# ShawnHymel/ei-keyword-spotting

Measured on AMD Instinct MI355X. Metric: 1s@16kHz clips/sec (MFCC+CNN), higher is better.
Workload: dtype f32

## Files before the change

### ei-keyword-spotting_amd/csrc/kws_fast.hip

```cpp
#include <atomic>

#include "kws_device.h"
#include "kws_fast.h"
#include "kws_bfly_m2k1.h"
#include "kws_fast_maxmin.h"
#if KWS_FAST_WPS >= 3
#define kws_fast_kernel kws_fast_kernel_w3
#define kws_launch_fast kws_launch_fast_w3
#define kws_launch_fast_prof kws_launch_fast_prof_w3
#endif
#include "kws_nn_int8_dev.h"

typedef float v4f __attribute__((ext_vector_type(4)));
#if KWS_FAST_WPS >= 3
#define KWS_OPAQUE3(v) asm volatile("" : "+v"(v))
#define KWS_LANE3(lane) ((int)__builtin_amdgcn_mbcnt_hi(~0u, __builtin_amdgcn_mbcnt_lo(~0u, 0u)))
#define KWS_FAST_SINK (shared + FP.sink_off)
#else
#define KWS_OPAQUE3(v) do { } while (0)
#define KWS_LANE3(lane) (lane)
#define KWS_FAST_SINK (F + FP.sink_off)
#endif
static_assert(KWS_FAST_ZF == KWS_ZF && KWS_FAST_WAVE == KWS_WAVE, "kws_fast.h mirrors kws_device.h");

// ... 514 lines not shown
    const unsigned inv = k.inv_ocp20;
    const int sstride = k.stage_stride, out_w = k.out_w, out_c = k.out_c, pool = k.pool, pstr = k.pool_stride;
    const float pmin = k.pool_min, pmax = k.pool_max;
    if (!pooled) {
        const int npad = out_cp - out_c;
        if (npad == 0) return;
        const unsigned pinv = k.inv_npad20;
        for (int i = lane; i < k.pool_w * npad; i += KWS_WAVE) {
            const int p = (int)(((unsigned)i * pinv) >> 20), c = out_c + (i - p * npad);
            img[p * out_stride + c] = 0.0f;
        }
        return;
    }
    for (int i0 = 0; i0 < items; i0 += 2 * KWS_WAVE) {
        float v[2][8];
        int p[2], c[2];
#pragma unroll
        for (int u = 0; u < 2; ++u) {
            const int i = min(i0 + u * KWS_WAVE + lane, items - 1);
            p[u] = (int)(((unsigned)i * inv) >> 20);
            c[u] = i - p[u] * out_cp;
            const float *sp = stage + p[u] * pstr * sstride + min(c[u], out_c - 1);
#pragma unroll
            for (int j = 0; j < 8; ++j) {
                const int r = (j < pool) ? min(p[u] * pstr + j, out_w - 1) : p[u] * pstr;
                v[u][j] = sp[(r - p[u] * pstr) * sstride];
            }
        }
#pragma unroll
        for (int u = 0; u < 2; ++u) {
            float m = v[u][0];
#pragma unroll
            for (int j = 1; j < 8; ++j) m = fast_max(m, v[u][j]);
            m = fast_clamp_u(m, pmin, pmax);
            if (i0 + u * KWS_WAVE + lane < items) img[p[u] * out_stride + c[u]] = c[u] < out_c ? m : 0.0f;
        }
    }
}

template <int TAPS>
__device__ __forceinline__ void fast_dw_t(const KwsFastBlock &k, const float *__restrict__ in, float *__restrict__ img,
                                          const float *__restrict__ shared, int lane, int out_stride, int out_cp)
{
    const int out_c = k.out_c, in_w = k.in_w, out_w = k.out_w, pad_left = k.pad_left, in_stride = k.in_stride, mult = k.mult;
    const bool pooled = k.pool > 1 || k.pool_stride > 1;
    const int n_seg = pooled ? k.pool_w : k.dw_nseg;
    const int seg_rows = pooled ? k.pool : k.dw_seg_rows, seg_step = pooled ? k.pool_stride : seg_rows;
    const int items = n_seg * out_cp;
    const unsigned inv = k.inv_ocp20;
    const float cmin = k.conv_min, cmax = k.conv_max, amin = k.add_min, amax = k.add_max, pmin = k.pool_min, pmax = k.pool_max;
    const bool has_add = k.has_add != 0;
    const float *wt = shared + k.w_off;
    for (int i = lane; i < items; i += KWS_WAVE) {
        const int seg = (int)(((unsigned)i * inv) >> 20), c = i - seg * out_cp, cc = min(c, out_c - 1);
        const float *col = in + (mult == 1 ? cc : cc / mult);
        float w[TAPS];
#pragma unroll
        for (int t = 0; t < TAPS; ++t) w[t] = wt[t * out_c + cc];
        const float bias = shared[k.bias_off + cc], addc = shared[k.addc_off + cc];
        const int r0 = seg * seg_step, r1 = min(r0 + seg_rows, out_w);
        auto fetch = [&](int row) { const float v = col[min(max(row, 0), in_w - 1) * in_stride]; return (unsigned)row < (unsigned)in_w ? v : 0.0f; };
        float x[TAPS + 3];
#pragma unroll
        for (int t = 0; t + 1 < TAPS; ++t) x[t] = fetch(r0 + t - pad_left);
        float m = -FLT_MAX;
        float *dst = img + c;
        for (int r = r0; r < r1; r += 4) {
#pragma unroll
            for (int e = 0; e < 4; ++e) x[TAPS - 1 + e] = fetch(r + e + TAPS - 1 - pad_left);
#pragma unroll
            for (int e = 0; e < 4; ++e) {
                float acc = 0.0f;
#pragma unroll
                for (int t = 0; t < TAPS; ++t) acc = __fmaf_rn(x[e + t], w[t], acc);
                float v = fminf(fmaxf(acc + bias, cmin), cmax);
                if (has_add) v = fminf(fmaxf(v + addc, amin), amax);
                const bool live = r + e < r1;
                if (pooled) m = live ? fmaxf(m, v) : m;
                else if (live) dst[(r + e) * out_stride] = c < out_c ? v : 0.0f;
            }
#pragma unroll
            for (int t = 0; t + 1 < TAPS; ++t) x[t] = x[t + 4];
        }
        if (pooled) dst[seg * out_stride] = c < out_c ? fminf(fmaxf(m, pmin), pmax) : 0.0f;
    }
}

__device__ __forceinline__ void fast_dwconv_any(const KwsFastBlock &k, const float *__restrict__ in, float *__restrict__ img,
                                                const float *__restrict__ shared, int lane, int out_stride, int out_cp)
{
    const int items = k.pool_w * out_cp, out_c = k.out_c, in_w = k.in_w, out_w = k.out_w, taps = k.taps, pad_left = k.pad_left;
    const int in_stride = k.in_stride, pool = k.pool, pstr = k.pool_stride, mult = k.mult;
    const unsigned inv = k.inv_ocp20;
    const float cmin = k.conv_min, cmax = k.conv_max, amin = k.add_min, amax = k.add_max, pmin = k.pool_min, pmax = k.pool_max;
    const bool has_add = k.has_add != 0;
    const float *wt = shared + k.w_off;
    for (int i = lane; i < items; i += KWS_WAVE) {
        const int p = (int)(((unsigned)i * inv) >> 20), c = i - p * out_cp, cc = min(c, out_c - 1);
        const float *col = in + (mult == 1 ? cc : cc / mult);
        const float bias = shared[k.bias_off + cc], addc = shared[k.addc_off + cc];
        float m = -FLT_MAX;
        for (int j = 0; j < pool; ++j) {
            const int r = p * pstr + j;
            if (r >= out_w) break;
            float acc = 0.0f;
            for (int tap = 0; tap < taps; ++tap) {
                const int row = r + tap - pad_left;
                if ((unsigned)row < (unsigned)in_w) acc = __fmaf_rn(col[row * in_stride], wt[tap * out_c + cc], acc);
            }
            float v = fminf(fmaxf(acc + bias, cmin), cmax);
            if (has_add) v = fminf(fmaxf(v + addc, amin), amax);
            m = fmaxf(m, v);
        }
        m = fminf(fmaxf(m, pmin), pmax);
        img[p * out_stride + c] = c < out_c ? m : 0.0f;
    }
}

__device__ __forceinline__ void fast_dwconv(const KwsFastBlock &k, const float *__restrict__ in, float *__restrict__ img,
                                            const float *__restrict__ shared, int lane, int out_stride, int out_cp)
{
    switch (k.taps) {
    case 1: fast_dw_t<1>(k, in, img, shared, lane, out_stride, out_cp); break;
    case 2: fast_dw_t<2>(k, in, img, shared, lane, out_stride, out_cp); break;
    case 3: fast_dw_t<3>(k, in, img, shared, lane, out_stride, out_cp); break;
    case 4: fast_dw_t<4>(k, in, img, shared, lane, out_stride, out_cp); break;
    case 5: fast_dw_t<5>(k, in, img, shared, lane, out_stride, out_cp); break;
    case 6: fast_dw_t<6>(k, in, img, shared, lane, out_stride, out_cp); break;
    case 7: fast_dw_t<7>(k, in, img, shared, lane, out_stride, out_cp); break;
    case 8: fast_dw_t<8>(k, in, img, shared, lane, out_stride, out_cp); break;
    default: fast_dwconv_any(k, in, img, shared, lane, out_stride, out_cp); break;
    }
}

template <int CR, int CG, bool DEFER, bool SPLIT = false, int SAFE = 0>
__device__ __forceinline__ float fast_cmvn(float *__restrict__ img, const float *__restrict__ cnt_tab, const int *__restrict__ upd, int fs,
                                           float inv_win, const float *__restrict__ guard_tab, float level, float abs_scale, bool silent, float sys_t2, int piv_row, const float *__restrict__ mref, bool c0_exact, int lane, int nfr, int ncep,
                                           const float *__restrict__ ext_tab, float *__restrict__ sink, int in_cp = 0)
{
    static_assert(!SPLIT || (DEFER && CG == 16), "the split store is written for column blocks of 16 and the deferred guard sum");
    static_assert(SAFE == 0 || (SPLIT && SAFE <= CR), "rows known to be live: the split form only");
    constexpr int NG = KWS_WAVE / CG;
    const int cgrp = min(lane / CG, NG - 1), cl = lane - (lane / CG) * CG;
    const bool lane_on = SPLIT || lane < NG * CG;
#define CMVN_ROW_LIVE(r0v, i) ((i) < SAFE || (r0v) + (i) < nfr)
#define CMVN_ROW(r0v, i) ((i) < SAFE ? (r0v) + (i) : min((r0v) + (i), nfr - 1))
    const int r0 = cgrp * CR;
    const int nfr8 = (nfr + 7) & ~7;
    const float *cnt = cnt_tab + cgrp * nfr8;
    float vacc = 0.0f;
    int u[CR - 1];
    int xo[KWS_FAST_CMVN_EXT];
    float we[KWS_FAST_CMVN_EXT], m0 = 0.0f;
#if KWS_FAST_WPS < 3
#pragma unroll
    for (int i = 0; i < CR - 1; ++i) u[i] = upd[min(r0 + i, nfr - 1)];
    if (ext_tab) {
        const float *ext = ext_tab + cgrp * (1 + 2 * KWS_FAST_CMVN_EXT);
        m0 = ext[0];
#pragma unroll
        for (int e = 0; e < KWS_FAST_CMVN_EXT; ++e) { xo[e] = __float_as_int(ext[1 + 2 * e]); we[e] = ext[2 + 2 * e]; }
    }
#endif
    for (int cb = 0; cb < ncep; cb += CG) {
#if KWS_FAST_WPS >= 3
        {
            int cg_ = cgrp;
            KWS_OPAQUE3(cg_);
            const int r0_ = cg_ * CR;
#pragma unroll
            for (int i = 0; i < CR - 1; ++i) u[i] = upd[CMVN_ROW(r0_, i)];
            if (ext_tab) {
                const float *ext = ext_tab + cg_ * (1 + 2 * KWS_FAST_CMVN_EXT);
                m0 = ext[0];
#pragma unroll
                for (int e = 0; e < KWS_FAST_CMVN_EXT; ++e) { xo[e] = __float_as_int(ext[1 + 2 * e]); we[e] = ext[2 + 2 * e]; }
            }
        }
#endif
        const int c = cb + cl;
        const bool act = lane_on && c < ncep && (SAFE > 0 || r0 < nfr);
        float *col = img + min(c, ncep - 1);
        const float piv = col[(ext_tab ? piv_row : min(r0 + CR / 2, nfr - 1)) * fs];
        const float4 gcol = ((const float4 *)guard_tab)[cb + cl];
        const bool is_c0 = c0_exact && cb + cl == 0;
        float g_abs = __fmaf_rn(gcol.y, level, gcol.x * abs_scale);
        if constexpr (SPLIT) g_abs = act ? g_abs : 0.0f;
        float g_rel = (cb + cl == 0 ? c0_exact : silent) ? gcol.w : gcol.z;
        float mr[CR];
#pragma unroll
        for (int i = 0; i < CR; ++i) mr[i] = (c0_exact && cb == 0) ? mref[CMVN_ROW(r0, i)] : 0.0f;
        float own[CR];
#pragma unroll
        for (int i = 0; i < CR; ++i) own[i] = col[CMVN_ROW(r0, i) * fs];
        float dl[CR - 1], da[CR - 1];
#pragma unroll
        for (int i = 0; i < CR - 1; ++i) { dl[i] = col[u[i] & 0xffff]; da[i] = col[(unsigned)u[i] >> 16]; }
        float S0 = 0.0f, S1 = 0.0f, Q0 = 0.0f, Q1 = 0.0f;
        if (ext_tab) {
            float xe[KWS_FAST_CMVN_EXT];
#pragma unroll
            for (int e = 0; e < KWS_FAST_CMVN_EXT; ++e) xe[e] = col[xo[e]];
            float T0 = 0.0f, T1 = 0.0f, U0 = 0.0f, U1 = 0.0f;
#pragma unroll
            for (int i = 0; i < CR; ++i) {
                const float d = (lane_on && CMVN_ROW_LIVE(r0, i)) ? own[i] - piv : 0.0f;
                if (i & 1) { T1 += d; U1 = __fmaf_rn(d, d, U1); } else { T0 += d; U0 = __fmaf_rn(d, d, U0); }
            }
            float T = T0 + T1, U = U0 + U1;
            float Tt = T, Ut = U;
#pragma unroll
            for (int g = 1; g < NG; ++g) {
                const int src = (cl + CG * ((cgrp + g) % NG)) << 2;
                Tt += __int_as_float(__builtin_amdgcn_ds_bpermute(src, __float_as_int(T)));
                Ut += __int_as_float(__builtin_amdgcn_ds_bpermute(src, __float_as_int(U)));
            }
            S0 = m0 * Tt; Q0 = m0 * Ut;
#pragma unroll
            for (int e = 0; e < KWS_FAST_CMVN_EXT; ++e) {
                const float d = xe[e] - piv, wd = we[e] * d;
                S1 += wd;
                Q1 = __fmaf_rn(wd, d, Q1);
            }
        } else
        for (int j0 = 0; j0 < nfr8; j0 += 8) {
            float x[8];
#pragma unroll
            for (int e = 0; e < 8; ++e) x[e] = col[min(j0 + e, nfr - 1) * fs];
            const float4 wa = *(const float4 *)(cnt + j0), wb = *(const float4 *)(cnt + j0 + 4);
            const float w[8] = { wa.x, wa.y, wa.z, wa.w, wb.x, wb.y, wb.z, wb.w };
#pragma unroll
            for (int e = 0; e < 8; e += 2) {
                const float d0 = x[e] - piv, d1 = x[e + 1] - piv;
                const float wd0 = w[e] * d0, wd1 = w[e + 1] * d1;
                S0 += wd0; S1 += wd1;
                Q0 = __fmaf_rn(wd0, d0, Q0); Q1 = __fmaf_rn(wd1, d1, Q1);
            }
        }
#pragma unroll
        for (int i = 0; i < CR - 1; ++i) { dl[i] -= piv; da[i] -= piv; }
        float S = S0 + S1, Q = Q0 + Q1;
        if constexpr (DEFER) {
            const float m0 = S * inv_win, v0 = fmaxf(__fmaf_rn(-m0, m0, Q * inv_win), 0.0f), am0 = m0 + piv;
            g_rel = (cb + cl != 0 && v0 < sys_t2 * (am0 * am0)) ? gcol.w : g_rel;
            if constexpr (SPLIT) g_rel = act ? g_rel : 0.0f;
        }
        float o[CR], gq[DEFER ? CR : 1];
#pragma unroll
        for (int i = 0; i < CR; ++i) {
            const float m = S * inv_win;
            float var = __fmaf_rn(-m, m, Q * inv_win);
            var = fmaxf(var, 0.0f);
            const float sd = __builtin_amdgcn_sqrtf(var);
            const float rstd = __builtin_amdgcn_rcpf(sd + FLT_EPSILON);
            const float gterm = __fmaf_rn(g_rel, fabsf(m + piv), g_abs) * rstd;
            if constexpr (DEFER) gq[i] = gterm;
            else vacc = (act && r0 + i < nfr) ? __fmaf_rn(gterm, gterm, vacc) : vacc;
            o[i] = (is_c0 ? own[i] - mr[i] : (own[i] - piv) - m) * rstd;
            if (i + 1 < CR) {
                S = (S + da[i]) - dl[i];
                Q = __fmaf_rn(da[i], da[i], Q);
                Q = __fmaf_rn(-dl[i], dl[i], Q);
            }
        }
        WAVE_SYNC();
        if constexpr (SPLIT) {
            _Float16 *const hcol = (_Float16 *)((char *)img + 4 * cb) + cl;
            const bool col_on = lane_on && c < in_cp;
            _Float16 *dst_i = col_on ? hcol + r0 * (2 * fs) : (_Float16 *)sink;
            const int dst_step = col_on ? 2 * fs : 0;
            float sc = c < ncep ? (float)(1 << KWS_SPLIT22_PRE_EXP) : 0.0f;
#pragma unroll
            for (int i = 0; i < CR; ++i) asm volatile("" : "+v"(o[i]));
#pragma unroll
            for (int i = 0; i < CR; ++i) {
                const bool live = CMVN_ROW_LIVE(r0, i);
                _Float16 hi, lo;
                const float d = kws_split22(o[i], sc, &hi, &lo);
                _Float16 *const dst = live ? dst_i : (_Float16 *)sink;
                dst[0] = hi;
                dst[KWS_FAST_PRE_LO / 2] = lo;
                dst_i += dst_step;
                sc = __fmaf_rn(d, 0.0f, sc);
                vacc = live ? __fmaf_rn(gq[i], gq[i], vacc) : vacc;
            }
            vacc = (SAFE > 0 || r0 < nfr) ? __fmaf_rn(sc, 0.0f, vacc) : vacc;
        } else {
#pragma unroll
        for (int i = 0; i < CR; ++i) {
            const int r = r0 + i;
            const bool live = act && r < nfr;
            *(live ? col + r * fs : sink) = o[i];
            if constexpr (DEFER) vacc = live ? __fmaf_rn(gq[i], gq[i], vacc) : vacc;
        }
        }
    }
    WAVE_SYNC();
    return vacc;
#undef CMVN_ROW_LIVE
#undef CMVN_ROW
}

#define KWS_FAST_NPHASE 20
#define FPH(i) do { if (PROF) { const long long now_ = clock64(); ph[i] += now_ - tlast; tlast = now_; } } while (0)

template <int NZ, int DG, bool PROF = false, bool FROM_CEP = false, bool NET = true, int QCP = 0, bool MFE = false>
__global__ __launch_bounds__(256 * KWS_FAST_WPS, KWS_FAST_WPS) void kws_fast_kernel(KwsDspPlan P, const KwsFastPlan *__restrict__ FPp, const int16_t *__restrict__ pcm, int n_clips,
                                                          float *__restrict__ scores, float *__restrict__ features,
                                                          int8_t *__restrict__ q_out, float in_scale, int in_zp,
                                                          int *__restrict__ flag_count, int *__restrict__ flag_list,
                                                          long long *__restrict__ prof_out = nullptr, const float *__restrict__ cep = nullptr,
                                                          const KwsNnPlan *__restrict__ QNp = nullptr, const int *__restrict__ sel = nullptr,
                                                          float *__restrict__ tap_logits = nullptr, int feat_in = 0)
{
    static_assert(QCP == 0 || !NET, "the int8 network follows the feature-emitting form");
    static_assert(!MFE || (!NET && QCP == 0 && !FROM_CEP && !PROF), "the MFE form is the spectral prefix: mel energies to HBM");
    const KwsFastPlan &FP = *FPp;
    extern __shared__ __attribute__((aligned(16))) float lds[];
    const int lane = threadIdx.x & (KWS_WAVE - 1), wave = __builtin_amdgcn_readfirstlane((int)(threadIdx.x >> 6));
    if (FROM_CEP && (int)blockIdx.x * (int)(blockDim.x >> 6) >= sel_count(sel, n_clips)) return;
    float *shared = lds;
    float *F = lds + FP.shared_floats + FP.q_floats + wave * FP.wave_floats;
    float *R1 = F + FP.f_floats;
    float *xw = R1, *pw = R1;
    for (int i = threadIdx.x; i < FP.shared_floats; i += blockDim.x) shared[i] = FP.shared_init[i];
    for (int i = lane; i < FP.r1_floats; i += KWS_WAVE) R1[i] = 0.0f;
    constexpr int Q_HEAD = 48 * 256, Q_WB1 = Q_HEAD + ((KWS_HEAD_BYTES + 15) & ~15), Q_WB2 = Q_WB1 + (QCP == 16 ? 4 : 16) * KWS_WAVE * 16,
                  Q_RQ = Q_WB2 + 4 * KWS_WAVE * 16;
    if constexpr (QCP != 0) {
        unsigned char *const qs = (unsigned char *)(lds + FP.shared_floats);
        const KwsNnPlan &QN = *QNp;
        for (int i = threadIdx.x * 4; i < QN.blk[0].out_c * 256; i += blockDim.x * 4) *(int *)(qs + i) = *(const int *)(QN.blk[0].add_lut + i);
        for (int i = threadIdx.x * 4; i < QN.blk[1].out_c * 256; i += blockDim.x * 4) *(int *)(qs + 32 * 256 + i) = *(const int *)(QN.blk[1].add_lut + i);
        (void)nn_head_stage(QN, qs + Q_HEAD);
        nn_mfma_stage_lds<QCP == 0 ? 16 : QCP>(QN, (v4i *)(qs + Q_WB1), (v4i *)(qs + Q_WB2), (int *)(qs + Q_RQ));
    }
    if constexpr (FROM_CEP)
        for (int i = lane; i < FP.wave_floats; i += KWS_WAVE) F[i] = 0.0f;
    __syncthreads();

    const int nfr = P.n_frames, ncep = P.n_cepstral, NF = 8 * DG;
    const int n_tail = (nfr >= KWS_FAST_MEL_CHUNK && (nfr & 7) != 0 && (nfr & 7) <= 2) ? (nfr & 7) : 0;
    const int n_pass = n_tail ? nfr / KWS_FAST_MEL_CHUNK : (nfr + KWS_FAST_MEL_CHUNK - 1) / KWS_FAST_MEL_CHUNK;
    const int fs = FP.fs;
    float *img = F;
    float *elog = F + nfr * fs;
    constexpr int NZ2 = DG > 4 ? KWS_FAST_NZ2 : 1;
    const float *dct_frag = shared + FP.dct_off;
    const int pstride = FP.pstride;
    const int n_waves = blockDim.x >> 6;
    const float pre_cof = P.pre_cof, pscale = kws_fast_pscale(P.inv_fft);
    const int frame_stride = P.frame_stride, n_samples = P.n_samples;
    const float *cnt_tab = shared + FP.cnt_off;
    const int *upd_tab = (const int *)(shared + FP.upd_off);
    const float *ext_tab = FP.ext_off >= 0 ? shared + FP.ext_off : nullptr;
    const float inv_win = FP.inv_win;
    const float *guard_tab = shared + (FROM_CEP ? FP.guard_cep_off : FP.guard_off);
    const int *pad_idx = (const int *)(shared + FP.pad_off);
    const int win_size = P.win_size, prow = nfr + 2 * P.pad;
    const int cr = FP.cr, n_blocks = FP.n_blocks, n_labels = FP.n_labels;
    (void)cr;
    long long ph[KWS_FAST_NPHASE] = { 0 }, tlast = PROF ? clock64() : 0;

    const int clip_stride = gridDim.x * n_waves;
    float *const stash = F + FP.stash_off;
    bool have_stash = false;
    const int n_sel = FROM_CEP ? sel_count(sel, n_clips) : n_clips;
#if KWS_FAST_WPS >= 3
    static_assert(!FROM_CEP, "the forms that start from cepstra are not built for three waves per SIMD");
    int *const tk = FP.tickets;
    int ni = 0;
    for (int ci = blockIdx.x * n_waves + wave; ci < n_sel; ci = ni) {
        int tv = 0;
        if (KWS_LANE3(lane) == 0) tv = __hip_atomic_fetch_add(tk, 1, __ATOMIC_RELAXED, __HIP_MEMORY_SCOPE_AGENT);
        const int clip = FROM_CEP ? sel_clip(sel, ci) : ci;
        const int next_ci = ci;
#else
    for (int ci = blockIdx.x * n_waves + wave; ci < n_sel; ci += clip_stride) {
        const int clip = FROM_CEP ? sel_clip(sel, ci) : ci;
        const int next_ci = ci + clip_stride;
        const int next_clip = ci + clip_stride < n_sel ? ci + clip_stride : -1;
#endif
        int lane_c = KWS_LANE3(lane);
        asm volatile("" : "+v"(lane_c));
        const int fl = lane_c & 7, fg = lane_c >> 3;
        const int nbA = (fl >> 2) + 4 * (fl & 3);
        const float a_c = P.tw[16].x, a_e = P.tw[32].x;
        const cf b1 = to_cf(P.tw[4 * fl]), b2 = to_cf(P.tw[8 * fl]), b3 = to_cf(P.tw[12 * fl]);
#if KWS_FAST_WPS >= 3
        const float *const twl_c = shared + FP.twl_off + 24 * fl, *const twl_s = shared + FP.twl_off + 192 + 16 * fl;
#else
        cf c1[4], c2[4], c3[4];
    #pragma unroll
        for (int a = 0; a < 4; ++a) { c1[a] = to_cf(P.tw[fl + 8 * a]); c2[a] = to_cf(P.tw[2 * (fl + 8 * a)]); c3[a] = to_cf(P.tw[3 * (fl + 8 * a)]); }
        cf stw[8];
    #pragma unroll
        for (int q = 0; q < 8; ++q) {
            const int k = fl + 8 * (q & 3) + 32 * (q >> 2);
            stw[q] = to_cf(P.stw[(k == 0 ? KWS_NC / 2 : k) - 1]);
        }
#endif
        const int xwr = fg * KWS_FAST_XS + 18 * fl;
        const int xrd = fg * KWS_FAST_XS + 2 * fl;
        const int partner = (lane_c & ~7) | ((8 - fl) & 7);
        const int half = lane_c >> 5, t = lane_c & 31;
        const int start1 = FP.tap_start1[lane_c], start2 = FP.tap_start2[lane_c];
        float lvl_sum = 0.0f;
        float w1[NZ], w2[NZ2];
    #pragma unroll
        for (int n = 0; n < NZ; ++n) w1[n] = FP.tap_w1[lane_c * KWS_FAST_NZ_MAX + n];
    #pragma unroll
        for (int n = 0; n < NZ2; ++n) w2[n] = FP.tap_w2[lane_c * KWS_FAST_NZ2 + n];
        int touched_a = 0, touched_b = 0;
        if constexpr (FROM_CEP) {
            const float *src = cep + (size_t)clip * (nfr * ncep);
            const int n_val = nfr * ncep;
            const unsigned inv = (1u << 20) / (unsigned)ncep + 1u;
            const int rr = P.ring_rows, rh = P.ring_head;
            auto ring = [&](int r) { const int t = r + rh; return (rr != 0 && r < rr) ? (t >= rr ? t - rr : t) : r; };
            auto trips = [&](int i_from, int i_to) {
                for (int i0 = i_from + lane; i0 - lane < i_to; i0 += 4 * KWS_WAVE) {
                    float v[4];
                    int dst[4];
#pragma unroll
                    for (int u = 0; u < 4; ++u) {
                        const int i = min(i0 + KWS_WAVE * u, n_val - 1);
                        const int r = (int)(((unsigned)i * inv) >> 20), c = i - r * ncep;
                        v[u] = src[ring(r) * ncep + c];
                        dst[u] = r * fs + c;
                    }
#pragma unroll
                    for (int u = 0; u < 4; ++u) if (i0 + KWS_WAVE * u < n_val) img[dst[u]] = v[u];
                }
            };
            trips(0, 4 * KWS_WAVE);
            if (next_ci < n_sel) {
                const char *nsrc = (const char *)(cep + (size_t)sel_clip(sel, next_ci) * n_val);
                const int nbytes = n_val * 4 - 4;
                touched_a = *(const int *)(nsrc + (min(128 * lane, nbytes) & ~3));
                touched_b = *(const int *)(nsrc + (min(128 * lane + 64, nbytes) & ~3));
            }
            trips(4 * KWS_WAVE, n_val);
            WAVE_SYNC();
        } else {
        const int16_t *xbase = pcm + (size_t)clip * n_samples;
        const int wrap_prev = (int)xbase[n_samples - 1];
        auto fetch = [&](int q, fast_i2 (&raw)[2][8]) {
            const int f = min(KWS_FAST_MEL_CHUNK * q + fg, nfr - 1);
            const int16_t *xf = xbase + (f * frame_stride + 2 * nbA - 2);
#pragma unroll
            for (int blk = 0; blk < 2; ++blk)
#pragma unroll
                for (int i = 0; i < 8; ++i) {
                    const int16_t *src = xf + (4 * blk + 32 * (i >> 1) + 128 * (i & 1));
                    if (blk == 0 && i == 0) src = src < xbase ? xbase : src;
                    raw[blk][i] = *(const fast_i2 *)src;
                }
        };
        auto touch = [&](int q) {
            const int f = min(KWS_FAST_MEL_CHUNK * q + fg, nfr - 1);
            return *(const int *)(xbase + (f * frame_stride + 32 * fl));
        };
        auto mel_phase = [&](int fbase, int nfc, int pairs, int adj1) {
            WAVE_SYNC();
            const int j2 = 32 + (lane_c & 7), sl2 = lane_c >> 3;
            const float *p1 = pw + 4 * half * pstride + start1, *p2 = pw + sl2 * pstride + start2;
            float macc[5] = { 1.0f, 1.0f, 1.0f, 1.0f, 1.0f };
#pragma unroll
            for (int s2 = 0; s2 < 4; s2 += 2) {
                if (s2 >= 2 * pairs) break;
                float xv[2][NZ];
#pragma unroll
                for (int s = 0; s < 2; ++s)
#pragma unroll
                    for (int n = 0; n < NZ; ++n) xv[s][n] = p1[(s2 + s) * pstride + n];
#pragma unroll
                for (int s = 0; s < 2; ++s) {
                    float acc = 0.0f;
#pragma unroll
                    for (int n = 0; n < NZ; ++n) acc = __fmaf_rn(xv[s][n], w1[n], acc);
                    macc[s2 + s] = acc;
                }
            }
            float acc2 = 0.0f;
            if (DG > 4) {
                float xv2[NZ2];
#pragma unroll
                for (int n = 0; n < NZ2; ++n) xv2[n] = p2[n];
#pragma unroll
                for (int n = 0; n < NZ2; ++n) acc2 = __fmaf_rn(xv2[n], w2[n], acc2);
            }
            macc[4] = acc2;
#pragma unroll
            for (int s = 0; s < 5; ++s) {
                const float a = macc[s] == 0.0f ? FLT_EPSILON : macc[s];
                macc[s] = MFE ? a : fast_log(a);
            }
#pragma unroll
            for (int s = 0; s < 4; ++s) {
                const int slot = 4 * half + s;
                if (slot < nfc && t < NF) img[(fbase + slot) * fs + t + (slot == 1 ? adj1 : 0)] = macc[s];
            }
            if (DG > 4 && sl2 < nfc && j2 < NF) img[(fbase + sl2) * fs + j2 + (sl2 == 1 ? adj1 : 0)] = macc[4];
        };
        fast_i2 nxt[2][8];
        fetch(0, nxt);
        int touched = touch(1);
#if KWS_FAST_WPS >= 3
        ni = clip_stride + __builtin_amdgcn_readfirstlane(tv);
        const int next_clip = ni < n_sel ? ni : -1;
#endif
        const bool pair_tail = n_tail == 1 && !have_stash && next_clip >= 0;
        int touched_tail = 0;
        const int16_t *const xnext = pcm + (size_t)max(next_clip, 0) * n_samples;
        if (pair_tail && lane_c < 8) touched_tail = *(const int *)(xnext + (nfr - 1) * frame_stride + 32 * lane_c);
        for (int q = 0; q < n_pass; ++q) {
            const int fbase = KWS_FAST_MEL_CHUNK * q;
            const int f = fbase + fg;
            const bool live = f < nfr;
            cf u[4][4];
            {
                cf z[2][8];
#pragma unroll
                for (int blk = 0; blk < 2; ++blk)
#pragma unroll
                    for (int i = 0; i < 8; ++i) z[blk][i] = fast_point(nxt[blk][i], pre_cof);
                if (f == 0 && fl == 0) {
                    fast_i2 v = nxt[0][0];
                    v.y = v.x;
                    v.x = wrap_prev << 16;
                    z[0][0] = fast_point(v, pre_cof);
                }
                fetch(q + 1, nxt);
                asm volatile("" : : "v"(touched));
                touched = touch(q + 2);
                FPH(0);
#pragma unroll
                for (int blk = 0; blk < 2; ++blk) {
                    cf sm[4], df[4];
#pragma unroll
                    for (int i = 0; i < 4; ++i) { sm[i] = cadd(z[blk][2 * i], z[blk][2 * i + 1]); df[i] = csub(z[blk][2 * i], z[blk][2 * i + 1]); }
                    bfly4_unit(sm[0], sm[1], sm[2], sm[3]);
                    bfly4_m2k1(df[0], df[1], df[2], df[3], a_c, a_e);
#pragma unroll
                    for (int i = 0; i < 4; ++i) { z[blk][2 * i] = sm[i]; z[blk][2 * i + 1] = df[i]; }
                }
#pragma unroll
                for (int rnd = 0; rnd < 2; ++rnd) {
#pragma unroll
                    for (int r = 0; r < 8; ++r) *(float2 *)(xw + xwr + 2 * r) = make_float2(z[rnd][r].r, z[rnd][r].i);
                    WAVE_SYNC();
#pragma unroll
                    for (int b = 0; b < 2; ++b)
#pragma unroll
                        for (int a = 0; a < 4; ++a) {
                            const float2 v = *(const float2 *)(xw + xrd + 18 * a + 72 * b);
                            u[a][2 * rnd + b].r = v.x; u[a][2 * rnd + b].i = v.y;
                        }
                    WAVE_SYNC();
                }
            }
#pragma unroll
            for (int b = 0; b < 4; ++b) bfly4(u[0][b], u[1][b], u[2][b], u[3][b], b1, b2, b3);
#pragma unroll
#if KWS_FAST_WPS >= 3
            for (int a = 0; a < 4; ++a) {
                const float4 c12 = *(const float4 *)(twl_c + 6 * a);
                const float2 c3v = *(const float2 *)(twl_c + 6 * a + 4);
                cf t1, t2, t3;
                t1.r = c12.x; t1.i = c12.y; t2.r = c12.z; t2.i = c12.w; t3.r = c3v.x; t3.i = c3v.y;
                bfly4(u[a][0], u[a][1], u[a][2], u[a][3], t1, t2, t3);
            }
            cf stw[8];
#pragma unroll
            for (int q = 0; q < 8; q += 2) {
                const float4 v = *(const float4 *)(twl_s + 2 * q);
                stw[q].r = v.x; stw[q].i = v.y; stw[q + 1].r = v.z; stw[q + 1].i = v.w;
            }
#else
            for (int a = 0; a < 4; ++a) bfly4(u[a][0], u[a][1], u[a][2], u[a][3], c1[a], c2[a], c3[a]);
#endif
            FPH(1);
            {
                float *prow = pw + fg * pstride;
                const bool lane0 = fl == 0;
                float esum = 0.0f;
#pragma unroll
                for (int qq = 0; qq < 8; ++qq) {
                    const int a = qq & 3, b = qq >> 2;
                    cf other;
                    other.r = __int_as_float(__builtin_amdgcn_ds_bpermute(partner << 2, __float_as_int(u[3 - a][3 - b].r)));
                    other.i = __int_as_float(__builtin_amdgcn_ds_bpermute(partner << 2, __float_as_int(u[3 - a][3 - b].i)));
                    cf fpk = u[a][b];
                    int k = fl + 8 * a + 32 * b;
                    {
                        const int o = qq == 0 ? 8 : 16 - qq;
                        other.r = lane0 ? u[o & 3][o >> 2].r : other.r;
                        other.i = lane0 ? u[o & 3][o >> 2].i : other.i;
                        if (qq == 0) { fpk.r = lane0 ? u[0][2].r : fpk.r; fpk.i = lane0 ? u[0][2].i : fpk.i; k = lane0 ? KWS_NC / 2 : k; }
                    }
                    cf fpnk; fpnk.r = other.r; fpnk.i = -other.i;
                    const cf f1k = cadd(fpk, fpnk), f2k = csub(fpk, fpnk);
                    const cf twv = cmul(f2k, stw[qq]);
                    cf lo, hi;
                    lo.r = f1k.r + twv.r;
                    lo.i = f1k.i + twv.i;
                    hi.r = f1k.r - twv.r;
                    hi.i = twv.i - f1k.i;
                    const float plo = __fmaf_rn(lo.r, lo.r, lo.i * lo.i);
                    const float phi = __fmaf_rn(hi.r, hi.r, hi.i * hi.i);
                    prow[k] = plo;
                    esum += (qq == 0 && lane0) ? 0.0f : plo;
                    esum += phi;
                    prow[KWS_NC - k] = phi;
                }
                if (fl == 0) {
                    const float dc = u[0][0].r + u[0][0].i, ny = u[0][0].r - u[0][0].i;
                    const float pdc = (dc * dc) * 4.0f, pny = (ny * ny) * 4.0f;
                    esum += pdc + pny;
                    prow[0] = pdc;
                }
                esum = oct_sum(esum) * pscale;
                if (fl == 0 && live) elog[f] = fast_log(esum == 0.0f ? FLT_EPSILON : esum);
            }
            FPH(2);

            mel_phase(fbase, min(KWS_FAST_MEL_CHUNK, nfr - fbase), 2, 0);
            WAVE_SYNC();
            FPH(3);
        }

        asm volatile("" : : "v"(touched_tail));
        if (n_tail == 1 && have_stash) {
            if (lane_c < NF) img[(nfr - 1) * fs + lane_c] = stash[lane_c];
            if (lane_c == 47) elog[nfr - 1] = stash[47];
            have_stash = false;
            WAVE_SYNC();
        } else if (n_tail) {
            const int16_t *const xb_t = (pair_tail && half == 1) ? xnext : xbase;
            const int ft = pair_tail ? nfr - 1 : KWS_FAST_MEL_CHUNK * n_pass + half;
            const bool live_t = ft < nfr;
            const int s0 = min(ft, nfr - 1) * frame_stride + 8 * t;
            const int4 rawv = *(const int4 *)(xb_t + s0);
            const int rawp = s0 == 0 ? wrap_prev : (int)xb_t[s0 - 1];
            const int k01 = t & 1, g01 = t >> 1, n0 = (g01 >> 2) + 4 * (g01 & 3), K2 = t & 7, G2 = t >> 3;
            const cf ta1 = to_cf(P.tw[16 * k01]), ta2 = to_cf(P.tw[32 * k01]), ta3 = to_cf(P.tw[48 * k01]);
            const cf tb1 = to_cf(P.tw[4 * K2]), tb2 = to_cf(P.tw[8 * K2]), tb3 = to_cf(P.tw[12 * K2]);
            const cf tc1 = to_cf(P.tw[t]), tc2 = to_cf(P.tw[2 * t]), tc3 = to_cf(P.tw[3 * t]);
            float *zb = R1 + 2 * pstride + half * KWS_ZF;
            {
                float y[8];
                float prev = (float)rawp;
                const int w[4] = { rawv.x, rawv.y, rawv.z, rawv.w };
#pragma unroll
                for (int i = 0; i < 4; ++i) {
                    const float lo = (float)(short)(w[i] & 0xffff), hi = (float)(w[i] >> 16);
                    const float pl = pre_cof * prev;
                    y[2 * i] = lo - pl;
                    const float ph_ = pre_cof * lo;
                    y[2 * i + 1] = hi - ph_;
                    prev = hi;
                }
                *(float4 *)(zb + 2 * zi(4 * t)) = make_float4(y[0], y[1], y[2], y[3]);
                *(float4 *)(zb + 2 * zi(4 * t) + 4) = make_float4(y[4], y[5], y[6], y[7]);
            }
            WAVE_SYNC();
            cf v[4];
            {
                cf la[4], lb[4];
#pragma unroll
                for (int i = 0; i < 4; ++i) { la[i] = ld_cf(zb, n0 + 16 * i); lb[i] = ld_cf(zb, n0 + 16 * i + 64); }
#pragma unroll
                for (int i = 0; i < 4; ++i) v[i] = k01 ? csub(la[i], lb[i]) : cadd(la[i], lb[i]);
            }
            bfly4(v[0], v[1], v[2], v[3], ta1, ta2, ta3);
            WAVE_SYNC();
#pragma unroll
            for (int i = 0; i < 4; ++i) st_cf(zb, 8 * g01 + k01 + 2 * i, v[i]);
            WAVE_SYNC();
#pragma unroll
            for (int i = 0; i < 4; ++i) v[i] = ld_cf(zb, 32 * G2 + K2 + 8 * i);
            bfly4(v[0], v[1], v[2], v[3], tb1, tb2, tb3);
#pragma unroll
            for (int i = 0; i < 4; ++i) st_cf(zb, 32 * G2 + K2 + 8 * i, v[i]);
            WAVE_SYNC();
#pragma unroll
            for (int i = 0; i < 4; ++i) v[i] = ld_cf(zb, t + 32 * i);
            bfly4(v[0], v[1], v[2], v[3], tc1, tc2, tc3);
#pragma unroll
            for (int i = 0; i < 4; ++i) st_cf(zb, t + 32 * i, v[i]);
            WAVE_SYNC();
            {
                const cf st1 = to_cf(P.stw[t]), st2 = to_cf(P.stw[t + 32]);
                cf fpk[2], fq[2];
#pragma unroll
                for (int rep = 0; rep < 2; ++rep) {
                    const int k = t + 1 + 32 * rep;
                    fpk[rep] = ld_cf(zb, k);
                    fq[rep] = ld_cf(zb, KWS_NC - k);
                }
                const float2 d0 = *(const float2 *)zb;
                float *prow = pw + half * pstride;
                float esum = 0.0f;
#pragma unroll
                for (int rep = 0; rep < 2; ++rep) {
                    const int k = t + 1 + 32 * rep;
                    const cf stw_ = rep ? st2 : st1;
                    cf fpnk; fpnk.r = fq[rep].r; fpnk.i = -fq[rep].i;
                    const cf f1k = cadd(fpk[rep], fpnk), f2k = csub(fpk[rep], fpnk);
                    const cf twv = cmul(f2k, stw_);
                    cf lo, hi;
                    lo.r = f1k.r + twv.r;
                    lo.i = f1k.i + twv.i;
                    hi.r = f1k.r - twv.r;
                    hi.i = twv.i - f1k.i;
                    const float plo = __fmaf_rn(lo.r, lo.r, lo.i * lo.i);
                    const float phi = __fmaf_rn(hi.r, hi.r, hi.i * hi.i);
                    if (k != KWS_NC / 2) {
                        esum += plo;
                        prow[k] = plo;
                    }
                    esum += phi;
                    prow[KWS_NC - k] = phi;
                }
                if (t == 0) {
                    const float dc = d0.x + d0.y, ny = d0.x - d0.y;
                    const float pdc = (dc * dc) * 4.0f, pny = (ny * ny) * 4.0f;
                    esum += pdc + pny;
                    prow[0] = pdc;
                }
                esum = half_wave_sum(esum) * pscale;
                if (t == 0 && live_t) *((pair_tail && half == 1) ? stash + 47 : elog + ft) = fast_log(esum == 0.0f ? FLT_EPSILON : esum);
            }
            mel_phase(KWS_FAST_MEL_CHUNK * n_pass, pair_tail ? 2 : n_tail, 1, pair_tail ? (int)(stash - img) - nfr * fs : 0);
            have_stash = pair_tail;
            WAVE_SYNC();
        }

        if constexpr (!MFE) {
            int lane_l = KWS_LANE3(lane);
            asm volatile("" : "+v"(lane_l));
            const int lm = lane_l & 15, lq = lane_l >> 4;
            float dB[DG][2][2];
#pragma unroll
            for (int g = 0; g < DG; ++g)
#pragma unroll
                for (int i = 0; i < 2; ++i)
#pragma unroll
                    for (int nt = 0; nt < 2; ++nt) dB[g][i][nt] = dct_frag[((g * 2 + i) * 2 + nt) * KWS_WAVE + lane_l];
            const float *arow = img + lm * fs + 2 * lq;
            float e0 = 0.0f;
            if (lane_l < nfr) e0 = elog[lane_l];
            v4f acc[4][2];
            __builtin_amdgcn_s_setprio(1);
#pragma unroll
            for (int rnd = 0; rnd < 2; ++rnd) {
                float2 a[2][DG];
#pragma unroll
                for (int m2 = 0; m2 < 2; ++m2)
#pragma unroll
                    for (int g = 0; g < DG; ++g) a[m2][g] = *(const float2 *)(arow + 16 * (2 * rnd + m2) * fs + 8 * g);
#pragma unroll
                for (int m2 = 0; m2 < 2; ++m2) { acc[2 * rnd + m2][0] = v4f{ 0.f, 0.f, 0.f, 0.f }; acc[2 * rnd + m2][1] = v4f{ 0.f, 0.f, 0.f, 0.f }; }
#pragma unroll
                for (int g = 0; g < DG; ++g) {
#pragma unroll
                    for (int m2 = 0; m2 < 2; ++m2)
#pragma unroll
                        for (int nt = 0; nt < 2; ++nt)
                            acc[2 * rnd + m2][nt] = __builtin_amdgcn_mfma_f32_16x16x4f32(a[m2][g].x, dB[g][0][nt], acc[2 * rnd + m2][nt], 0, 0, 0);
#pragma unroll
                    for (int m2 = 0; m2 < 2; ++m2)
#pragma unroll
                        for (int nt = 0; nt < 2; ++nt)
                            acc[2 * rnd + m2][nt] = __builtin_amdgcn_mfma_f32_16x16x4f32(a[m2][g].y, dB[g][1][nt], acc[2 * rnd + m2][nt], 0, 0, 0);
                }
            }
            __builtin_amdgcn_s_setprio(0);
            WAVE_SYNC();
            float *const sink = KWS_FAST_SINK + lane_l;
#if KWS_FAST_WPS >= 3
            float *dbase[2];
            int dstep[2];
#pragma unroll
            for (int nt = 0; nt < 2; ++nt) {
                const int n = 16 * nt + lm;
                const bool col_ok = n <= NF / 2 && n > 0;
                dbase[nt] = col_ok ? img + 4 * lq * fs + n : sink;
                dstep[nt] = col_ok ? fs : 0;
            }
            auto dct_store = [&](auto full_c) {
                constexpr int FULL = decltype(full_c)::value;
#pragma unroll
                for (int mt = 0; mt < 4; ++mt)
#pragma unroll
                    for (int i = 0; i < 4; ++i) {
                        const bool row_ok = mt < FULL || 16 * mt + 4 * lq + i < nfr;
#pragma unroll
                        for (int nt = 0; nt < 2; ++nt) {
                            float *const dst = dbase[nt] + (16 * mt + i) * dstep[nt];
                            *(row_ok ? dst : sink) = acc[mt][nt][i];
                        }
                        lvl_sum += row_ok ? fabsf(acc[mt][0][i]) : 0.0f;
                    }
            };
            if (nfr >= 48) dct_store(std::integral_constant<int, 3>()); else dct_store(std::integral_constant<int, 0>());
            if (lane_l < nfr) img[lane_l * fs] = e0;
#else
#pragma unroll
            for (int mt = 0; mt < 4; ++mt)
#pragma unroll
                for (int nt = 0; nt < 2; ++nt) {
                    const int n = 16 * nt + lm;
                    const bool col_ok = n <= NF / 2 && n > 0;
#pragma unroll
                    for (int i = 0; i < 4; ++i) {
                        const int r = 16 * mt + 4 * lq + i;
                        *((col_ok && r < nfr) ? img + r * fs + n : sink) = acc[mt][nt][i];
                    }
                }
            if (lane_l < nfr) img[lane_l * fs] = e0;
#pragma unroll
            for (int mt = 0; mt < 4; ++mt)
#pragma unroll
                for (int i = 0; i < 4; ++i) lvl_sum += (16 * mt + 4 * lq + i < nfr) ? fabsf(acc[mt][0][i]) : 0.0f;
#endif
            lvl_sum = lm == 0 ? lvl_sum : 0.0f;
            WAVE_SYNC();
        }
        FPH(4);
        }

        float *fout = features ? features + (size_t)clip * (nfr * ncep) : nullptr;
        int8_t *qclip = q_out ? q_out + (size_t)clip * (nfr * ncep) : nullptr;
        int8_t *const act1 = (int8_t *)R1;
        float vlane = 0.0f;
        int lane_m = KWS_LANE3(lane);
        asm volatile("" : "+v"(lane_m));
        float *const csink = KWS_FAST_SINK + lane_m;
        bool c0_exact = false, silent = false;
        int n_silent = 0;
        int piv_row = 0;
        const bool feats_given = FROM_CEP && feat_in != 0;
        if constexpr (!MFE) if (!feats_given) {
            const bool on = lane_m < nfr;
            const float x0 = img[min(lane_m, nfr - 1) * fs];
            const unsigned long long smask = __ballot(on && x0 == fast_log(FLT_EPSILON));
            silent = smask != 0ull;
            piv_row = silent ? __builtin_ctzll(smask) : 0;
            if constexpr (!FROM_CEP) {
                if (silent && FP.sil_off >= 0) {
                    const int half_nf = min(NF / 2, ncep - 1);
                    const float sv = shared[FP.sil_off + min(lane_m + 1, 31)];
                    float *const dst = img + 1 + lane_m;
                    for (unsigned long long mm = smask; mm != 0ull; mm &= mm - 1ull) {
                        const int r = __builtin_ctzll(mm);
                        if (lane_m < half_nf) dst[r * fs] = sv;
                    }
                    n_silent = __popcll(smask);
                    WAVE_SYNC();
                }
            }
            const float mu = wave_sum(on ? x0 : 0.0f) * FP.c0_inv_rows;
            const float d0 = on ? x0 - mu : 0.0f;
            const float sd0 = __builtin_amdgcn_sqrtf(wave_sum(d0 * d0) * FP.c0_inv_rows);
            const float top = wave_max(on ? fabsf(x0) : 0.0f);
            c0_exact = silent || !(FP.c0_factor * sd0 >= __fmaf_rn(FP.c0_rel, top, FP.c0_abs));
        }
        if (c0_exact) {
            constexpr int PS = 260;
            float *pc = R1;
            for (int p = lane_m; p < prow; p += KWS_WAVE) {
                int prw[4];
                float pvv[4];
#pragma unroll
                for (int sft = 0; sft < 4; ++sft) prw[sft] = pad_idx[min(p + sft, prow - 1)];
#pragma unroll
                for (int sft = 0; sft < 4; ++sft) pvv[sft] = img[prw[sft] * fs];
#pragma unroll
                for (int sft = 0; sft < 4; ++sft) pc[sft * PS + p] = pvv[sft];
            }
            WAVE_SYNC();
            const int r = min(lane_m, nfr - 1);
            const float4 *pv = (const float4 *)(pc + (r & 3) * PS + (r & ~3));
            float sum = 0.0f;
            int q = 0;
            const int nq = win_size >> 2;
            for (; q + 4 <= nq; q += 4) {
                float4 v[4];
#pragma unroll
                for (int e = 0; e < 4; ++e) v[e] = pv[q + e];
#pragma unroll
                for (int e = 0; e < 4; ++e) { sum += v[e].x; sum += v[e].y; sum += v[e].z; sum += v[e].w; }
            }
            for (; q < nq; ++q) { const float4 v = pv[q]; sum += v.x; sum += v.y; sum += v.z; sum += v.w; }
            {
                const float4 v = pv[q];
                const int rem = win_size & 3;
                if (rem > 0) sum += v.x;
                if (rem > 1) sum += v.y;
                if (rem > 2) sum += v.z;
            }
            if (lane_m < nfr) elog[lane_m] = __fdiv_rn(sum, (float)win_size);
            WAVE_SYNC();
        }
        if (PROF) { const long long now_ = clock64(); ph[19] += now_ - tlast; }
        if constexpr (QCP != 0) {
            const int z1 = (int)((unsigned)(QNp->blk[0].in_zp & 0xff) * 0x01010101u);
            for (int i = lane_m; i < KWS_A1_ROWS * (QCP / 4); i += KWS_WAVE) ((int *)act1)[i] = z1;
            WAVE_SYNC();
        }
        float gV = 0.0f;
        if constexpr (!MFE) {
          if (feats_given) gV = FP.v_net_feat;
          else {
            float level = FROM_CEP ? 0.0f : wave_sum(lvl_sum) * FP.lvl_inv, abs_scale = 1.0f;
            if (!FROM_CEP && n_silent > 0) {
                const float live = (float)(nfr - n_silent), rows = (float)nfr;
                level = live > 0.0f ? fmaxf(__fmaf_rn(level, rows, (float)n_silent * fast_log(FLT_EPSILON)), 0.0f) / live : 0.0f;
                abs_scale = __builtin_amdgcn_sqrtf(live / rows);
                level *= abs_scale;
            }
#if KWS_FAST_WPS >= 3
            constexpr bool TWO_COPIES = !(NZ == 8 && DG == 5);
            if (TWO_COPIES && nfr >= 3 * 13 + 9) vlane = fast_cmvn<13, 16, true, true, 9>(img, cnt_tab, upd_tab, fs, inv_win, guard_tab, level, abs_scale, silent, FP.sys_t2, piv_row, elog, c0_exact, lane_m, nfr, ncep, ext_tab, csink, FP.blk[0].in_cp);
            else vlane = fast_cmvn<13, 16, true, true>(img, cnt_tab, upd_tab, fs, inv_win, guard_tab, level, abs_scale, silent, FP.sys_t2, piv_row, elog, c0_exact, lane_m, nfr, ncep, ext_tab, csink, FP.blk[0].in_cp);
#else
            if (cr == 13) vlane = fast_cmvn<13, 16, QCP == 0>(img, cnt_tab, upd_tab, fs, inv_win, guard_tab, level, abs_scale, silent, FP.sys_t2, piv_row, elog, c0_exact, lane_m, nfr, ncep, ext_tab, csink);
            else vlane = fast_cmvn<17, 20, QCP == 0>(img, cnt_tab, upd_tab, fs, inv_win, guard_tab, level, abs_scale, silent, FP.sys_t2, piv_row, elog, c0_exact, lane_m, nfr, ncep, ext_tab, csink);
#endif
            gV = __int_as_float(__builtin_amdgcn_readfirstlane(__float_as_int(wave_sum(vlane) + FP.v_net)));
          }
        }
        if constexpr (!NET) {
            if (!MFE && !(gV * fmaxf(FP.g_c1 * 0.0625f, FP.g_c2) <= 1.0f)) {
                if (lane == 0) flag_list[atomicAdd(flag_count, 1)] = clip;
            }
        }
        if constexpr (!NET) {
            const unsigned inv = (1u << 20) / (unsigned)ncep + 1u;
            const int q_pad = QCP != 0 ? QNp->blk[0].pad_left : 0;
            for (int i = lane; i < nfr * ncep; i += KWS_WAVE) {
                const int r = (int)(((unsigned)i * inv) >> 20), c = i - r * ncep;
                const float o = img[r * fs + c];
                if (fout) fout[i] = o;
                if (QCP != 0 || qclip) {
                    const int8_t qb = quantize_feature(o, in_scale, in_zp);
                    if (qclip) qclip[i] = qb;
                    if constexpr (QCP != 0) act1[(r + q_pad) * QCP + c] = qb;
                }
            }
            WAVE_SYNC();
        }
        FPH(5);
        if constexpr (QCP != 0) {
            const KwsNnPlan &QN = *QNp;
            int8_t *const act2 = (int8_t *)F;
            int *const vec = (int *)(F + KWS_A2_ROWS * 8);
            const int z2 = (int)((unsigned)(QN.blk[1].in_zp & 0xff) * 0x01010101u);
            for (int i = lane; i < KWS_A2_ROWS * 8; i += KWS_WAVE) ((int *)act2)[i] = z2;
            WAVE_SYNC();
            unsigned char *const qs = (unsigned char *)(lds + FP.shared_floats);
            const NnMfmaLds<QCP> qctx = nn_mfma_lds_ctx<QCP>(QN, (const v4i *)(qs + Q_WB1), (const v4i *)(qs + Q_WB2), (const int *)(qs + Q_RQ), lane);
            const NnHeadTab q_head = nn_head_tab(qs + Q_HEAD);
            const NnTaps no_taps = { nullptr, 0, nullptr, nullptr, nullptr, nullptr };
            __builtin_amdgcn_s_setprio(1);
            nn_mfma_clip<QCP>(qctx, QN, q_head, act1, act2, vec, (const int8_t *)qs, (const int8_t *)qs + 32 * 256, lane, clip, scores, no_taps);
            __builtin_amdgcn_s_setprio(0);
            WAVE_SYNC();
        }
        if constexpr (FROM_CEP) asm volatile("" : : "v"(touched_a), "v"(touched_b));
        if constexpr (!NET) continue;
        else {

        float *cur = F, *oth = R1;
#if KWS_FAST_WPS >= 3
        int lane_n = KWS_LANE3(lane);
        asm volatile("" : "+v"(lane_n));
        int ws_off = FP.sink_off + lane_n;
        asm volatile("" : "+v"(ws_off));
        float *const wsink = shared + ws_off;
#else
        float *const wsink = KWS_FAST_SINK + lane;
        int lane_n = lane;
        asm volatile("" : "+v"(lane_n));
#endif
        for (int b = 0; b < n_blocks; ++b) {
            const KwsFastBlock &k = FP.blk[b];
            int lane_b = lane_n;
            KWS_OPAQUE3(lane_b);
            const bool last = b + 1 == n_blocks;
            const int o_stride = last ? k.out_c : FP.blk[b + 1].in_stride;
            const int o_cp = last ? k.out_c : FP.blk[b + 1].in_cp;
            const bool pooled = k.pool > 1 || k.pool_stride > 1;
            float *stage = pooled ? cur : oth;
            const int sstride = pooled ? k.stage_stride : o_stride;
            long long t_loop = 0, t_pre = 0, *tl = (PROF && b == 0) ? &t_loop : nullptr, *tp = (PROF && b == 0) ? &t_pre : nullptr;
            if (k.dw) {
                fast_dwconv(k, cur, oth, shared, lane_b, o_stride, o_cp);
                WAVE_SYNC();
                float *tmp = cur; cur = oth; oth = tmp;
                if (PROF && b > 0) { const long long now_ = clock64(); ph[12 + b] += now_ - tlast; }
                FPH(6 + (b > 0));
                continue;
            }
            float cscale = 1.0f;
            if (k.hconv) {
                const int zo = FP.zero_off;
                const bool bgl = k.h_b_off < 0;
                const bool pre = KWS_FAST_WPS >= 3 && b == 0;
                if (bgl && k.n_tiles == 1 && k.m_tiles == 1 && k.h_ks <= 8) cscale = fast_conv_small_h<1>(k, cur, stage, sstride, shared, zo, lane_b, wsink, pre);
                else
                switch ((k.m_tiles > 2 ? 4 : k.m_tiles) * 4 + k.n_tiles) {
                case 4 * 4 + 2: cscale = bgl ? fast_conv_tiles_h<4, 2, true>(k, cur, stage, sstride, shared, zo, lane_b, wsink, pre) : fast_conv_tiles_h<4, 2, false, (DG > 4)>(k, cur, stage, sstride, shared, zo, lane_b, wsink, pre); break;
                case 4 * 4 + 1: cscale = bgl ? fast_conv_tiles_h<4, 1, true>(k, cur, stage, sstride, shared, zo, lane_b, wsink, pre) : fast_conv_tiles_h<4, 1, false>(k, cur, stage, sstride, shared, zo, lane_b, wsink, pre); break;
                case 2 * 4 + 2: cscale = bgl ? fast_conv_tiles_h<2, 2, true>(k, cur, stage, sstride, shared, zo, lane_b, wsink, pre) : fast_conv_tiles_h<2, 2, false>(k, cur, stage, sstride, shared, zo, lane_b, wsink, pre); break;
                case 2 * 4 + 1: cscale = bgl ? fast_conv_tiles_h<2, 1, true>(k, cur, stage, sstride, shared, zo, lane_b, wsink, pre) : fast_conv_tiles_h<2, 1, false>(k, cur, stage, sstride, shared, zo, lane_b, wsink, pre); break;
                case 1 * 4 + 2: cscale = bgl ? fast_conv_tiles_h<1, 2, true>(k, cur, stage, sstride, shared, zo, lane_b, wsink, pre) : fast_conv_tiles_h<1, 2, false>(k, cur, stage, sstride, shared, zo, lane_b, wsink, pre); break;
                default: cscale = bgl ? fast_conv_tiles_h<1, 1, true>(k, cur, stage, sstride, shared, zo, lane_b, wsink, pre) : fast_conv_tiles_h<1, 1, false>(k, cur, stage, sstride, shared, zo, lane_b, wsink, pre); break;
                }
            } else
            switch (k.m_tiles * 4 + k.n_tiles) {
            case 4 * 4 + 2: fast_conv_tiles<4, 2>(k, cur, stage, sstride, shared, lane_b, wsink, tl, tp); break;
            case 4 * 4 + 1: fast_conv_tiles<4, 1>(k, cur, stage, sstride, shared, lane_b, wsink); break;
            case 3 * 4 + 2: fast_conv_tiles<3, 2>(k, cur, stage, sstride, shared, lane_b, wsink, tl, tp); break;
            case 3 * 4 + 1: fast_conv_tiles<3, 1>(k, cur, stage, sstride, shared, lane_b, wsink); break;
            case 2 * 4 + 2: fast_conv_tiles<2, 2>(k, cur, stage, sstride, shared, lane_b, wsink); break;
            case 2 * 4 + 1: fast_conv_tiles<2, 1>(k, cur, stage, sstride, shared, lane_b, wsink); break;
            case 1 * 4 + 2: fast_conv_tiles<1, 2>(k, cur, stage, sstride, shared, lane_b, wsink); break;
            default: fast_conv_tiles<1, 1>(k, cur, stage, sstride, shared, lane_b, wsink); break;
            }
            WAVE_SYNC();
            if (PROF && b == 0 && t_loop != 0) { ph[9] += t_loop - t_pre; ph[10] += clock64() - t_loop; ph[11] += t_pre - tlast; }
            if (k.fpool) fast_pool_finish(k, stage, oth, shared, lane_b, o_stride, o_cp, cscale);
            else fast_pool(k, stage, oth, lane_b, o_stride, o_cp, pooled);
            WAVE_SYNC();
            float *tmp = cur; cur = oth; oth = tmp;
            if (PROF && b > 0) { const long long now_ = clock64(); ph[12 + b] += now_ - tlast; }
            FPH(6 + (b > 0));
        }
        {
            const int fc_in = FP.fc_in, fc_out = FP.fc_out;
            const int sh = fc_out > 1 ? 32 - __builtin_clz(fc_out - 1) : 0;
            const int S = KWS_WAVE >> sh, unit = lane_n >> (6 - sh), sl = lane_n & (S - 1), uc = min(unit, fc_out - 1);
            const float *wfc = shared + FP.fc_w_off + uc * fc_in;
            float tot = 0.0f, tot1 = 0.0f;
            int i = sl;
            for (; i + S < fc_in; i += 2 * S) { tot = __fmaf_rn(cur[i], wfc[i], tot); tot1 = __fmaf_rn(cur[i + S], wfc[i + S], tot1); }
            if (i < fc_in) tot = __fmaf_rn(cur[i], wfc[i], tot);
            tot = group_sum(tot + tot1, S) + shared[FP.fc_b_off + uc];
            tot = fast_clamp_u(tot, FP.fc_min, FP.fc_max);
            const bool on = unit < fc_out;
            if (tap_logits && on && sl == 0) tap_logits[(size_t)clip * n_labels + unit] = tot;
            const float mx = wave_max(on ? tot : -FLT_MAX);
            const float e = expf((tot - mx) * FP.beta);
// ... 148 lines not shown
```

Baseline: 57.73 million.

## Streamline mel pass with byte-offset fetches, full-chunk fast path, and deferred energy log

For the three-waves-per-SIMD build, sample fetches now use precomputed byte offsets clamped once per pass instead of recomputing frame pointers, and full mel chunks take a branch-free path that loads all filter inputs up front and stores without per-slot guards. The per-frame energy log is moved out of the FFT pass into the DCT stage, where one lane per frame computes it. The pass loop body is also wrapped in a lambda. The aim is to cut address arithmetic, predication and register pressure in the hot loop, at the cost of more code paths and possible changes in register allocation.

```diff
diff --git a/ei-keyword-spotting_amd/csrc/kws_fast.hip b/ei-keyword-spotting_amd/csrc/kws_fast.hip
--- a/ei-keyword-spotting_amd/csrc/kws_fast.hip
+++ b/ei-keyword-spotting_amd/csrc/kws_fast.hip
@@ -840,6 +840,20 @@
 }
 
 #define KWS_FAST_NPHASE 20
+#ifndef KWS_FAST_FULL_PASS
+#define KWS_FAST_FULL_PASS (KWS_FAST_WPS >= 3)
+#endif
+#ifndef KWS_FAST_SOFS
+#define KWS_FAST_SOFS (KWS_FAST_WPS >= 3)
+#endif
+#ifndef KWS_FAST_LATE_ELOG
+#define KWS_FAST_LATE_ELOG (KWS_FAST_WPS >= 3)
+#endif
+#if KWS_FAST_LATE_ELOG
+#define KWS_FAST_ELOG(e) (e)
+#else
+#define KWS_FAST_ELOG(e) fast_log((e) == 0.0f ? FLT_EPSILON : (e))
+#endif
 #define FPH(i) do { if (PROF) { const long long now_ = clock64(); ph[i] += now_ - tlast; tlast = now_; } } while (0)
 
 template <int NZ, int DG, bool PROF = false, bool FROM_CEP = false, bool NET = true, int QCP = 0, bool MFE = false>
@@ -983,7 +997,27 @@
         } else {
         const int16_t *xbase = pcm + (size_t)clip * n_samples;
         const int wrap_prev = (int)xbase[n_samples - 1];
+#if KWS_FAST_SOFS
+        const char *const xb = (const char *)xbase;
+        const int pass_bytes = 2 * KWS_FAST_MEL_CHUNK * frame_stride;
+        const int sofs0 = 2 * (min(fg, nfr - 1) * frame_stride + 2 * nbA), sofs_last = 2 * ((nfr - 1) * frame_stride + 2 * nbA);
+        auto sofs = [&](int q) { return min(sofs0 + q * pass_bytes, sofs_last); };
+        const int tch_d = 64 * fl - 4 * nbA;
+        auto fetch_at = [&](auto first_c, int so, fast_i2 (&raw)[2][8]) {
+#pragma unroll
+            for (int blk = 0; blk < 2; ++blk)
+#pragma unroll
+                for (int i = 0; i < 8; ++i) {
+                    const unsigned o = (decltype(first_c)::value && blk == 0 && i == 0) ? (unsigned)max(so, 4) : (unsigned)so;
+                    raw[blk][i] = *(const fast_i2 *)(xb + o + (2 * (4 * blk + 32 * (i >> 1) + 128 * (i & 1)) - 4));
+                }
+        };
+        constexpr bool SOFS = !PROF;
+#endif
         auto fetch = [&](int q, fast_i2 (&raw)[2][8]) {
+#if KWS_FAST_SOFS
+            if constexpr (SOFS) { fetch_at(std::false_type(), sofs(q), raw); return; }
+#endif
             const int f = min(KWS_FAST_MEL_CHUNK * q + fg, nfr - 1);
             const int16_t *xf = xbase + (f * frame_stride + 2 * nbA - 2);
 #pragma unroll
@@ -996,14 +1030,51 @@
                 }
         };
         auto touch = [&](int q) {
+#if KWS_FAST_SOFS
+            if constexpr (SOFS) return *(const int *)(xb + (unsigned)(sofs(q) + tch_d));
+#endif
             const int f = min(KWS_FAST_MEL_CHUNK * q + fg, nfr - 1);
             return *(const int *)(xbase + (f * frame_stride + 32 * fl));
         };
-        auto mel_phase = [&](int fbase, int nfc, int pairs, int adj1) {
+        auto mel_phase = [&](auto full_c, int fbase, int nfc, int pairs, int adj1) {
             WAVE_SYNC();
             const int j2 = 32 + (lane_c & 7), sl2 = lane_c >> 3;
             const float *p1 = pw + 4 * half * pstride + start1, *p2 = pw + sl2 * pstride + start2;
             float macc[5] = { 1.0f, 1.0f, 1.0f, 1.0f, 1.0f };
+            if constexpr (decltype(full_c)::value) {
+                float xv[4][NZ], xv2[NZ2];
+                if (DG > 4) {
+#pragma unroll
+                    for (int n = 0; n < NZ2; ++n) xv2[n] = p2[n];
+                }
+#pragma unroll
+                for (int s = 0; s < 4; ++s)
+#pragma unroll
+                    for (int n = 0; n < NZ; ++n) xv[s][n] = p1[s * pstride + n];
+#pragma unroll
+                for (int s = 0; s < 4; ++s) {
+                    float acc = 0.0f;
+#pragma unroll
+                    for (int n = 0; n < NZ; ++n) acc = __fmaf_rn(xv[s][n], w1[n], acc);
+                    macc[s] = acc;
+                }
+                float acc2 = 0.0f;
+                if (DG > 4) {
+#pragma unroll
+                    for (int n = 0; n < NZ2; ++n) acc2 = __fmaf_rn(xv2[n], w2[n], acc2);
+                }
+                macc[4] = acc2;
+#pragma unroll
+                for (int s = 0; s < 5; ++s) {
+                    const float a = macc[s] == 0.0f ? FLT_EPSILON : macc[s];
+                    macc[s] = MFE ? a : fast_log(a);
+                }
+                float *const d1 = img + (fbase + 4 * half) * fs + t;
+#pragma unroll
+                for (int s = 0; s < 4; ++s) d1[s * fs] = macc[s];
+                if (DG > 4) img[(fbase + sl2) * fs + j2] = macc[4];
+                return;
+            }
 #pragma unroll
             for (int s2 = 0; s2 < 4; s2 += 2) {
                 if (s2 >= 2 * pairs) break;
@@ -1042,6 +1113,10 @@
             if (DG > 4 && sl2 < nfc && j2 < NF) img[(fbase + sl2) * fs + j2 + (sl2 == 1 ? adj1 : 0)] = macc[4];
         };
         fast_i2 nxt[2][8];
+#if KWS_FAST_SOFS
+        if constexpr (SOFS) fetch_at(std::true_type(), sofs0, nxt);
+        else
+#endif
         fetch(0, nxt);
         int touched = touch(1);
 #if KWS_FAST_WPS >= 3
@@ -1052,7 +1127,11 @@
         int touched_tail = 0;
         const int16_t *const xnext = pcm + (size_t)max(next_clip, 0) * n_samples;
         if (pair_tail && lane_c < 8) touched_tail = *(const int *)(xnext + (nfr - 1) * frame_stride + 32 * lane_c);
+#if KWS_FAST_WPS >= 3
+        auto pass_body = [&](int q) {
+#else
         for (int q = 0; q < n_pass; ++q) {
+#endif
             const int fbase = KWS_FAST_MEL_CHUNK * q;
             const int f = fbase + fg;
             const bool live = f < nfr;
@@ -1159,14 +1238,23 @@
                     prow[0] = pdc;
                 }
                 esum = oct_sum(esum) * pscale;
-                if (fl == 0 && live) elog[f] = fast_log(esum == 0.0f ? FLT_EPSILON : esum);
+                if (fl == 0 && live) elog[f] = KWS_FAST_ELOG(esum);
             }
             FPH(2);
 
-            mel_phase(fbase, min(KWS_FAST_MEL_CHUNK, nfr - fbase), 2, 0);
+#if KWS_FAST_FULL_PASS
+            if (nfr - fbase >= KWS_FAST_MEL_CHUNK) mel_phase(std::true_type(), fbase, KWS_FAST_MEL_CHUNK, 2, 0);
+            else
+#endif
+            mel_phase(std::false_type(), fbase, min(KWS_FAST_MEL_CHUNK, nfr - fbase), 2, 0);
             WAVE_SYNC();
             FPH(3);
-        }
+#if KWS_FAST_WPS >= 3
+        };
+        for (int q = 0; q < n_pass; ++q) pass_body(q);
+#else
+        }
+#endif
 
         asm volatile("" : : "v"(touched_tail));
         if (n_tail == 1 && have_stash) {
@@ -1268,9 +1356,9 @@
                     prow[0] = pdc;
                 }
                 esum = half_wave_sum(esum) * pscale;
-                if (t == 0 && live_t) *((pair_tail && half == 1) ? stash + 47 : elog + ft) = fast_log(esum == 0.0f ? FLT_EPSILON : esum);
-            }
-            mel_phase(KWS_FAST_MEL_CHUNK * n_pass, pair_tail ? 2 : n_tail, 1, pair_tail ? (int)(stash - img) - nfr * fs : 0);
+                if (t == 0 && live_t) *((pair_tail && half == 1) ? stash + 47 : elog + ft) = KWS_FAST_ELOG(esum);
+            }
+            mel_phase(std::false_type(), KWS_FAST_MEL_CHUNK * n_pass, pair_tail ? 2 : n_tail, 1, pair_tail ? (int)(stash - img) - nfr * fs : 0);
             have_stash = pair_tail;
             WAVE_SYNC();
         }
@@ -1288,7 +1376,11 @@
                     for (int nt = 0; nt < 2; ++nt) dB[g][i][nt] = dct_frag[((g * 2 + i) * 2 + nt) * KWS_WAVE + lane_l];
             const float *arow = img + lm * fs + 2 * lq;
             float e0 = 0.0f;
+#if KWS_FAST_LATE_ELOG
+            if (lane_l < nfr) { const float en = elog[lane_l]; e0 = fast_log(en == 0.0f ? FLT_EPSILON : en); }
+#else
             if (lane_l < nfr) e0 = elog[lane_l];
+#endif
             v4f acc[4][2];
             __builtin_amdgcn_s_setprio(1);
 #pragma unroll
```

After: 58.81 million, median of 6. +1.9%, better.
